# skhu101/SHERF

Hardware: NVIDIA B200
Metric: ray_samples_per_sec (higher is better)
Workload: dtype bf16x3 (bf16 hi/lo split products on tcgen05 kind::f16, 16 significand bits per operand, fp32 accumulate) in every linear layer

## Files before the change

include/sherf_b200.h:

```cpp
#ifndef SHERF_B200_H
#define SHERF_B200_H

#include <stddef.h>
#include <stdint.h>

#ifdef __cplusplus
extern "C" {
#endif

#define SHERF_ABI_VERSION 5
#if defined(__GNUC__)
#define SHERF_API __attribute__((visibility("default")))
#else
#define SHERF_API
#endif
#define SHERF_NUM_JOINTS 24
#define SHERF_NUM_LEVELS 3

enum {
  SHERF_OK = 0,
  SHERF_E_INVALID = -1,
  SHERF_E_SCRATCH = -2,
  SHERF_E_CUDA = -3,
  SHERF_E_UNSUPPORTED = -4
// ... 237 lines not shown
                                            int32_t* bins_out , void* stream);

SHERF_API int sherf_debug_linear(int precision, const float* A, int lda, const float* W, const float* bias, float* Y, int ldy,
                                 int M, int N, int K, int act, void* scratch, size_t scratch_bytes, void* stream);

SHERF_API void sherf_debug_set_trace(long long* device_buf);

SHERF_API const char* sherf_last_error(void);
SHERF_API int sherf_abi_version(void);
SHERF_API int64_t sherf_last_launch_count(void);
SHERF_API int64_t sherf_last_importance_point_count(void);
SHERF_API void sherf_set_profiling(int enabled);
SHERF_API float sherf_last_stage_ms(int stage);
SHERF_API float sherf_last_host_us(int part);
SHERF_API int sherf_nn_list_stats(double* out);

#ifdef __cplusplus
}
#endif
#endif
```

sherf_b200/_lib.py:

```python
from __future__ import annotations

import ctypes as C
import os

from . import build as _build

c_float_p = C.c_void_p
c_int_p = C.c_void_p

MLP_FP32, MLP_TF32, MLP_TF32X3, MLP_BF16X3 = 0, 1, 2, 3
ABI_VERSION = 5


class SherfSmplModel(C.Structure):
    _fields_ = [('v_template', c_float_p), ('shapedirs', c_float_p), ('posedirs', c_float_p), ('j_regressor', c_float_p),
                ('weights', c_float_p), ('parents', C.c_int32 * 24), ('n_verts', C.c_int32)]


class SherfPose(C.Structure):
    _fields_ = [('poses', c_float_p), ('shapes', c_float_p), ('R', c_float_p), ('Th', c_float_p)]


class SherfFrame(C.Structure):
    _fields_ = [('target', SherfPose), ('canonical', SherfPose), ('obs', SherfPose), ('vertices', c_float_p),
# ... 63 lines not shown


class SherfSparseEncoderGrads(C.Structure):
    _fields_ = [('weight', c_float_p * 13), ('bn_weight', c_float_p * 13), ('bn_bias', c_float_p * 13)]


class SherfObservation(C.Structure):
    _fields_ = [('obs', SherfPose), ('canonical', SherfPose), ('obs_vertices', c_float_p), ('t_vertices', c_float_p), ('obs_K', c_float_p),
                ('obs_R', c_float_p), ('obs_T', c_float_p), ('faces', c_int_p), ('last_face', c_int_p), ('n_faces', C.c_int32),
                ('reserved', C.c_int32), ('obs_img', c_float_p), ('img_h', C.c_int32), ('img_w', C.c_int32), ('obs_feat', c_float_p),
                ('feat_ch', C.c_int32), ('feat_h', C.c_int32), ('feat_w', C.c_int32), ('reserved2', C.c_int32), ('proj_w', c_float_p),
                ('proj_b', c_float_p)]


EXPORTS = ['sherf_render_backward_after_forward', 'sherf_sparse_encoder_train_scratch_bytes', 'sherf_sparse_encode_train', 'sherf_sparse_encode_backward', 'sherf_prepare_observation_backward', 'sherf_backward_scratch_bytes', 'sherf_render_backward', 'sherf_smpl_vertices', 'sherf_count_survivors', 'sherf_observation_scratch_bytes', 'sherf_prepare_observation', 'sherf_debug_set_trace', 'sherf_sparse_encoder_scratch_bytes', 'sherf_sparse_encode', 'sherf_generate_rays', 'sherf_debug_sample_importance', 'sherf_debug_linear', 'sherf_scratch_bytes', 'sherf_render_forward', 'sherf_lbs_transforms', 'sherf_depth_range', 'sherf_last_error',
           'sherf_abi_version', 'sherf_last_launch_count', 'sherf_last_importance_point_count', 'sherf_set_profiling', 'sherf_last_stage_ms', 'sherf_last_host_us', 'sherf_nn_list_stats']

_lib = None


def lib_path() -> str:
    return _build.LIB_PATH


def load():
    global _lib
    if _lib is not None:
        return _lib
    path = lib_path()
    if not os.path.exists(path):
        raise RuntimeError(f'{path} not found: build it with `python -m sherf_b200.build` (or __graft_entry__.build()); '
# ... 53 lines not shown
    lib.sherf_observation_scratch_bytes.restype = C.c_size_t
    lib.sherf_observation_scratch_bytes.argtypes = [C.c_int32]
    lib.sherf_prepare_observation.restype = C.c_int
    lib.sherf_prepare_observation.argtypes = [C.POINTER(SherfSmplModel), C.POINTER(SherfObservation), C.c_void_p, C.c_void_p, C.c_void_p,
                                              C.c_void_p, C.POINTER(C.c_int32), C.c_void_p, C.c_void_p, C.c_size_t, C.c_void_p]
    lib.sherf_debug_set_trace.argtypes = [C.c_void_p]
    lib.sherf_last_error.restype = C.c_char_p
    lib.sherf_abi_version.restype = C.c_int
    lib.sherf_last_launch_count.restype = C.c_int64
    lib.sherf_last_importance_point_count.restype = C.c_int64
    lib.sherf_set_profiling.argtypes = [C.c_int]
    lib.sherf_last_stage_ms.restype = C.c_float
    lib.sherf_last_stage_ms.argtypes = [C.c_int]
    lib.sherf_nn_list_stats.restype = C.c_int
    lib.sherf_nn_list_stats.argtypes = [C.POINTER(C.c_double)]
    lib.sherf_last_host_us.restype = C.c_float
    lib.sherf_last_host_us.argtypes = [C.c_int]
    if lib.sherf_abi_version() != ABI_VERSION:
        raise RuntimeError('libsherf_b200.so ABI version mismatch')
    _lib = lib
    return lib


def check(rc: int):
    if rc != 0:
        raise RuntimeError(f'sherf_b200 error {rc}: {load().sherf_last_error().decode()}')
```

sherf_b200/csrc/api.cu:

```cuda
#include "common.cuh"
#include "stages.cuh"
#include <cstdarg>
#include <cstdio>
#include <cstring>
#include <cstdlib>
#include <vector>
#include <chrono>

namespace sherf {

thread_local LaunchCounter g_launches;
thread_local bool g_pack_plan_only = false;
static thread_local char g_err[512] = "";
static thread_local int64_t g_last_launches = 0;
static thread_local int64_t g_last_fine_points = 0;
static thread_local int g_profiling = 0;
static thread_local float g_stage_ms[8] = {0, 0, 0, 0, 0, 0, 0, 0};
static thread_local FrameTables g_last_ft{};
static thread_local float g_host_us[4] = {0, 0, 0, 0};
static inline double now_us() { return std::chrono::duration<double, std::micro>(std::chrono::steady_clock::now().time_since_epoch()).count(); }

void set_error(const char* fmt, ...) {
  va_list ap;
  va_start(ap, fmt);
  vsnprintf(g_err, sizeof(g_err), fmt, ap);
  va_end(ap);
}

constexpr int kMaxCell = 1 << 18;

bool nn_lists_enabled() {
  const char* e = getenv("SHERF_NN_LEGACY");
  return !(e && atoi(e) != 0);
}
int nn_list_cap() {
  const char* e = getenv("SHERF_NN_LIST_CAP");
  const int k = e ? atoi(e) : kNnlCap;
  return k < 1 ? 1 : (k > kNnlCap ? kNnlCap : k);
}
static size_t chunk_cap_limit() {
  static size_t cap = 0;
  if (!cap) {
    const char* e = getenv("SHERF_CHUNK_CAP");
    const long v = e ? atol(e) : 0;
    cap = v >= 128 ? (size_t)(v / 128 * 128) : (size_t)(1 << 19);
  }
  return cap;
}

struct Arena {
  char* base; size_t size; size_t off; bool dry;
  template <typename T> T* take(size_t n) {
    off = (off + 255) & ~(size_t)255;
// ... 7 lines not shown
  FrameTables ft;
  float* planes_cl; float* feat_cl; float* vol_cl[3];
  int* sample_vid; int* ray_count; int* block_sums; int* ray_start; int64_t* total;
  int* point_sample; int* point_vid;
  float* sigma; float* rgb;
  float* fine_depths; int* sample_vid_f; int* ray_count_f; int* ray_start_f; int64_t* total_f; int* point_sample_f; int* point_vid_f;
  float* sigma_f; float* rgb_f;
  float* packed_w;
  float* canon_w;
  unsigned char* fused_blob; float* fused_bias; float* xf_blob; float* ff_blob;
  unsigned char* pp_blob; float* pp_bias; unsigned char* pp_xv;
  unsigned char* xb_blob; unsigned char* fr_blob;
  float* chunk;
  float* gather2;
  float* lbs_joints; float* lbs_pf;
};

static int chunk_cap(int N, int S, int SF) {
  const size_t NS = (size_t)N * (S > SF ? S : SF);
  return (int)((NS < chunk_cap_limit()) ? ((NS + 127) / 128 * 128) : chunk_cap_limit());
}

static size_t carve(Arena& a, const SherfScene& sc, int N, int S, int SF, int V, Layout& L) {
  const size_t NS = (size_t)N * S, NF = (size_t)N * SF;
  FrameTables& ft = L.ft;
  ft.fc = a.take<FrameConst>(1);
  ft.A = a.take<float>(3 * kJoints * 16);
  ft.joints = a.take<float>(3 * kJoints * 3);
  ft.posefeat = a.take<float>(3 * kPoseFeat);
  ft.poff = a.take<float>((size_t)3 * V * 3);
  ft.soff = a.take<float>((size_t)2 * V * 3);
  ft.verts_smpl = a.take<float>((size_t)V * 3);
  ft.T1 = a.take<VertexWarp>(V);
  ft.T3 = a.take<VertexWarp>(V);
  ft.g1_cell_start = a.take<int>(kMaxCell + 1);
  ft.g3_cell_start = a.take<int>(kMaxCell + 1);
  ft.g_cursor = a.take<int>((size_t)2 * kMaxCell);
  ft.g_block_sums = a.take<int>((size_t)2 * (kMaxCell / 1024 + 2));
  ft.g_total = a.take<int64_t>(2);
  ft.g1_verts = a.take<float4>(V);
  ft.g3_verts = a.take<float4>(V);
  ft.g1_occ = a.take<unsigned char>(kMaxCell);
  ft.maxcell = kMaxCell;
  ft.nnl_on = nn_lists_enabled() ? 1 : 0;
  ft.nnl_cap = nn_list_cap();
  ft.nnl_count = a.take<int>(4);
  ft.nnl_cand = a.take<unsigned char>((size_t)kMaxCell * kNnlSub3);
  for (int g = 0; g < 2; ++g) {
    ft.nnl_slot[g] = a.take<int>(kMaxCell);
    ft.nnl_slot_cell[g] = a.take<int>(kNnlSlots);
    ft.nnl_len[g] = a.take<int>((size_t)kNnlSlots * kNnlSub3);
    ft.nnl_ent[g] = a.take<float4>((size_t)kNnlSlots * kNnlSub3 * kNnlCap);
  }
  L.lbs_joints = a.take<float>(kJoints * 3);
  L.lbs_pf = a.take<float>(kPoseFeat);
  L.planes_cl = a.take<float>((size_t)3 * sc.plane_ch * sc.plane_h * sc.plane_w);
  L.feat_cl = a.take<float>((size_t)sc.feat_ch * sc.feat_h * sc.feat_w);
  for (int l = 0; l < 3; ++l)
    L.vol_cl[l] = a.take<float>((size_t)sc.vol_ch[l] * sc.vol_dim[l][0] * sc.vol_dim[l][1] * sc.vol_dim[l][2]);
  L.sample_vid = a.take<int>(NS);
// ... 190 lines not shown
    SHERF_CUDA_OK(cudaMemcpy(len.data(), ft.nnl_len[g], sizeof(int) * (size_t)nsub, cudaMemcpyDeviceToHost));
    double sum = 0.0, mx = 0.0, over = 0.0;
    for (int i = 0; i < nsub; ++i) {
      if (len[i] < 0) over += 1.0;
      else { sum += len[i]; mx = len[i] > mx ? len[i] : mx; }
    }
    out[1 + 4 * g] = nsub;
    out[2 + 4 * g] = nsub > over ? sum / (nsub - over) : 0.0;
    out[3 + 4 * g] = mx;
    out[4 + 4 * g] = nsub ? over / nsub : 0.0;
  }
  out[9] = ft.nnl_cap;
  return SHERF_OK;
}

size_t sherf_scratch_bytes(const SherfScene* scene, int32_t n_rays, int32_t n_samples, int32_t n_importance, int32_t n_verts) {
  if (!scene || n_rays <= 0 || n_samples < 2 || n_importance < 0 || n_verts <= 0) return 0;
  Arena a{nullptr, 0, 0, true};
  Layout L;
  return carve(a, *scene, n_rays, n_samples, n_importance, n_verts, L) + 512;
}

static int validate(const SherfSmplModel* smpl, const SherfFrame* fr, const SherfScene* sc, const SherfWeights* w,
                    const SherfRays* rays, const SherfOptions* opts, const SherfOut* out) {
  if (!smpl || !fr || !sc || !w || !rays || !opts || !out) { set_error("null argument struct"); return SHERF_E_INVALID; }
  if (rays->n_rays <= 0 || rays->n_samples < 2 || rays->n_samples > 256) {
    set_error("n_rays must be > 0 and 2 <= n_samples <= 256 (got %d, %d)", rays->n_rays, rays->n_samples);
    return SHERF_E_INVALID;
  }
  if ((int64_t)rays->n_rays * rays->n_samples >= (1LL << 31)) { set_error("n_rays * n_samples must be < 2^31"); return SHERF_E_INVALID; }
// ... 32 lines not shown

int sherf_render_forward(const SherfSmplModel* smpl, const SherfFrame* frame, const SherfScene* scene,
                         const SherfWeights* weights, const SherfRays* rays, const SherfOptions* opts, const SherfOut* out,
                         const SherfDebug* dbg, void* scratch, size_t scratch_bytes, void* stream, int64_t* n_points_out) {
  g_err[0] = 0;
  const double t_enter = now_us();
  RC(validate(smpl, frame, scene, weights, rays, opts, out));
  const int N = rays->n_rays, S = rays->n_samples, SF = rays->n_importance, V = smpl->n_verts;
  cudaStream_t st = (cudaStream_t)stream;
  Arena a{(char*)scratch, scratch_bytes, 0, false};
  const size_t mis = ((size_t)a.base) & 255;
  if (mis) { a.base += 256 - mis; a.size -= 256 - mis; }
  Layout L;
  const size_t need = carve(a, *scene, N, S, SF, V, L);
  if (!scratch || need > a.size) { set_error("scratch arena too small: need %zu bytes, have %zu", need, scratch_bytes); return SHERF_E_SCRATCH; }
  g_launches.n = 0;
  g_last_fine_points = 0;
  StageTimer tm;
  tm.init(g_profiling != 0, st);
  g_tm = &tm;
  struct Guard {
    cudaStream_t st; bool forked = false, joined = false;
    ~Guard() {
      g_tm = nullptr;
      if (forked && !joined && g_side.s) { cudaEventRecord(g_side.ldone, g_side.s); cudaStreamWaitEvent(st, g_side.ldone, 0); }
    }
  } guard;
  guard.st = st;

  const bool side = !getenv("SHERF_NO_PROLOGUE_OVERLAP") && g_side.ensure() == 0;
// ... 548 lines not shown
```

sherf_b200/csrc/common.cuh:

```cuda
#pragma once
#include <cuda_runtime.h>
#include <stdint.h>
#include <stddef.h>
#include <string.h>
#include "../../include/sherf_b200.h"

namespace sherf {

constexpr int kJoints = 24;
constexpr int kPoseFeat = 207;
constexpr float kPi2 = 1.57079632679489661923f;

struct GridDesc {
  float origin[3];
  float inv_cell;
  float cell;
  int dim[3];
  int ncell;
};

constexpr int kNnlSub = 2;
constexpr int kNnlSub3 = kNnlSub * kNnlSub * kNnlSub;
constexpr int kNnlCap = 64;
constexpr int kNnlSlots = 6144;

struct NnLists {
  const int* slot;
  const int* len;
  const float4* ent;
  const unsigned char* cand;
};

__device__ __forceinline__ bool nnl_cell(const GridDesc& g, float qx, float qy, float qz, int& cell, int& sub) {
  const float tx = (qx - g.origin[0]) * g.inv_cell, ty = (qy - g.origin[1]) * g.inv_cell, tz = (qz - g.origin[2]) * g.inv_cell;
  const int cx = (int)floorf(tx), cy = (int)floorf(ty), cz = (int)floorf(tz);
  if (cx < 0 || cx >= g.dim[0] || cy < 0 || cy >= g.dim[1] || cz < 0 || cz >= g.dim[2]) return false;
  cell = (cz * g.dim[1] + cy) * g.dim[0] + cx;
  const int sx = min((int)((tx - (float)cx) * (float)kNnlSub), kNnlSub - 1);
  const int sy = min((int)((ty - (float)cy) * (float)kNnlSub), kNnlSub - 1);
  const int sz = min((int)((tz - (float)cz) * (float)kNnlSub), kNnlSub - 1);
  sub = (sz * kNnlSub + sy) * kNnlSub + sx;
  return true;
}

__device__ __forceinline__ int nnl_index(const GridDesc& g, const int* __restrict__ slot, float qx, float qy, float qz) {
  int cell, sub;
  if (!nnl_cell(g, qx, qy, qz, cell, sub)) return -1;
  const int sl = slot[cell];
  return sl < 0 ? sl - 1 : sl * kNnlSub3 + sub;
}

struct __align__(16) VertexWarp {
  float Rinv[9];
  float t[3];
  float off0[3];
  float off1[3];
  float off2[3];
  float Af[12];
  float pad[3];
};
static_assert(sizeof(VertexWarp) == 36 * 4, "VertexWarp must be 144 B");

struct FrameConst {
  float R_tgt[9], Th_tgt[3];
// ... 84 lines not shown
  int* g_cursor;
  int* g_block_sums;
  int64_t* g_total;
  float4* g1_verts;
  float4* g3_verts;
  unsigned char* g1_occ;
  int maxcell;
  int nnl_on;
  int nnl_cap;
  int* nnl_slot[2];
  int* nnl_slot_cell[2];
  int* nnl_count;
  int* nnl_len[2];
  float4* nnl_ent[2];
  unsigned char* nnl_cand;
  NnLists lists(int g) const {
    return nnl_on ? NnLists{nnl_slot[g], nnl_len[g], nnl_ent[g], g == 0 ? nnl_cand : nullptr} : NnLists{nullptr, nullptr, nullptr, nullptr};
  }
};
bool nn_lists_enabled();
int nn_list_cap();

int run_prologue_frame(const SherfFrame& frame, const FrameTables& ft, cudaStream_t st);
int run_prologue_cull(const SherfSmplModel& smpl, const SherfFrame& frame, const SherfRays& rays, const SherfOptions& opts,
                      const FrameTables& ft, cudaStream_t st);
int run_prologue_tables(const SherfSmplModel& smpl, const SherfFrame& frame, const FrameTables& ft, cudaStream_t st);
int run_lbs_only(const SherfSmplModel& smpl, const SherfPose& pose, float* A_out, float* joints_tmp, float* pf_tmp, cudaStream_t st);
int run_depth_range(const SherfRays& rays, FrameConst* fc, cudaStream_t st);
int run_exclusive_scan(const int* cnt, int n, int* block_sums, int* start, int64_t* total_dev, cudaStream_t st);

}
```

sherf_b200/csrc/cull.cu:

```cuda
#include "common.cuh"

namespace sherf {

__device__ __forceinline__ void nn_27(const GridDesc& g, const int* __restrict__ cell_start, const float4* __restrict__ gv,
                                      float qx, float qy, float qz, int cx, int cy, int cz, float& best, int& best_id) {
  const int x0 = max(cx - 1, 0), x1 = min(cx + 1, g.dim[0] - 1);
  for (int z = max(cz - 1, 0); z <= min(cz + 1, g.dim[2] - 1); ++z) {
    for (int y = max(cy - 1, 0); y <= min(cy + 1, g.dim[1] - 1); ++y) {
      const int row = (z * g.dim[1] + y) * g.dim[0];
      const int b = cell_start[row + x0], e = cell_start[row + x1 + 1];
      for (int k = b; k < e; ++k) {
        const float4 v = gv[k];
        const float d2 = dist2_xyz(qx, qy, qz, v.x, v.y, v.z);
        const int id = __float_as_int(v.w);
        if (d2 < best || (d2 == best && id < best_id)) { best = d2; best_id = id; }
      }
    }
  }
}

__device__ __forceinline__ void cull_query(const FrameConst& fc, const float* __restrict__ origins, const float* __restrict__ dirs, int n,
                                           float t, float q[3]) {
  float p[3];
  p[0] = __fsub_rn(mul_add_sep(t, dirs[n * 3], origins[n * 3]), fc.Th_tgt[0]);
// ... 84 lines not shown
  __syncthreads();
  const GridDesc& g = fc.g1;
  const int count = *queue_count;
  if (cand_out && blockIdx.x == 0 && threadIdx.x == 0) *cand_out = count;
  for (int j = blockIdx.x * blockDim.x + threadIdx.x; j < count; j += gridDim.x * blockDim.x) {
    const int s = queue[j];
    const int n = s / S, i = s - n * S;
    const float t = depths ? depths[s] : sample_depth(nearv[n], farv[n], i, S);
    float q[3];
    cull_query(fc, origins, dirs, n, t, q);
    float best = 3.0e38f;
    int bid = 0x7fffffff;
    const float qx = q[0], qy = q[1], qz = q[2];
    const int li = nl.slot ? nnl_index(g, nl.slot, qx, qy, qz) : -1;
    const int ln = li >= 0 ? nl.len[li] : -1;
    if (ln >= 0) {
      const float4* e = nl.ent + (size_t)li * kNnlCap;
      for (int k = 0; k < ln; ++k) {
        const float4 v = e[k];
        const float d2 = dist2_xyz(qx, qy, qz, v.x, v.y, v.z);
        const int id = __float_as_int(v.w);
        if (d2 < best || (d2 == best && id < bid)) { best = d2; bid = id; }
      }
    } else {
      const int cx = grid_coord(q[0], g.origin[0], g.inv_cell, g.dim[0]);
      const int cy = grid_coord(q[1], g.origin[1], g.inv_cell, g.dim[1]);
      const int cz = grid_coord(q[2], g.origin[2], g.inv_cell, g.dim[2]);
      nn_27(g, cell_start, gv, qx, qy, qz, cx, cy, cz, best, bid);
    }
    const int vid = best < thr ? bid : -1;
// ... 107 lines not shown
```

sherf_b200/csrc/front_fused.cu:

```cuda
#include "common.cuh"
#include "stages.cuh"
#include "umma.cuh"
#include <cuda_bf16.h>
#include <cstdlib>

namespace sherf {

namespace fr {
constexpr uint32_t kLboA = 2080;
constexpr uint32_t kChunkHalf = 4 * kLboA;
constexpr uint32_t kChunk = 2 * kChunkHalf;
constexpr int kSlots = 3;
constexpr uint32_t kLboF = 2048;
constexpr uint32_t kF3d = kSlots * kChunk;
constexpr uint32_t kWr = kF3d + 12 * kLboF;
constexpr uint32_t kWrBlock = 4096;
constexpr uint32_t kWp = kWr + 3 * kWrBlock;
constexpr uint32_t kWpStage = 12288;
constexpr uint32_t kSmemBytes = kWp + 2 * kWpStage;
constexpr uint32_t kD1 = 0, kD2 = 96, kF3dLo = 192;
constexpr int kThreads = 512;
}

struct FrontArgs {
// ... 184 lines not shown
        const int k3 = l4 < 3 ? l4 : 0;
        const float ck = k3 == 0 ? cn[0] : (k3 == 1 ? cn[1] : cn[2]);
        const float gnv = ((ck - fc.spb_min[k3]) / 0.005f) / fc.out_sh[2 - k3] * 2.f - 1.f;
        const float cnv = 2.f * (ck - fc.twb_min[k3]) / (fc.twb_max[k3] - fc.twb_min[k3]) - 1.f;
        if (l4 < 3) { s_pt[gi][l4] = gnv; s_pt[gi][3 + l4] = cnv; }
        pu = u; pv = v;
      }
      if (act) {
        if (l4 < 3) {
          P.geo[(size_t)lp * 8 + l4] = l4 == 0 ? cn[0] : (l4 == 1 ? cn[1] : cn[2]);
          P.geo[(size_t)lp * 8 + 3 + l4] = l4 == 0 ? cdir[0] : (l4 == 1 ? cdir[1] : cdir[2]);
        } else {
          P.geo[(size_t)lp * 8 + 6] = 0.f;
          P.geo[(size_t)lp * 8 + 7] = 0.f;
        }
        if (DBG && l4 == 0 && gp < P.dbg_max) {
          if (P.dbg_vid3) P.dbg_vid3[gp] = vid3;
          if (P.dbg_can) { P.dbg_can[gp * 3] = cn[0]; P.dbg_can[gp * 3 + 1] = cn[1]; P.dbg_can[gp * 3 + 2] = cn[2]; }
          if (P.dbg_cdir) { P.dbg_cdir[gp * 3] = cdir[0]; P.dbg_cdir[gp * 3 + 1] = cdir[1]; P.dbg_cdir[gp * 3 + 2] = cdir[2]; }
          if (P.dbg_uv) { P.dbg_uv[gp * 2] = u; P.dbg_uv[gp * 2 + 1] = v; }
        }
      }
    }
    __syncwarp();

    int offT[2] = {-1, -1}, offI = -1;
    float wT[2] = {0.f, 0.f}, wI = 0.f;
    const float* pt = s_pt[gi];
#pragma unroll 1
    for (int c = 0; c < 12; ++c) {
// ... 248 lines not shown
  if (G.np <= 0) return SHERF_OK;
  if (!G.t_vertices) { set_error("internal: the front kernel needs the seeded canonical-vertex search"); return SHERF_E_INVALID; }
  FrontArgs a;
  a.G = G; a.wblob = blob; a.bp = w.proj_b; a.br = w.reproj_b; a.tok = tok;
  { const char* e = getenv("SHERF_FRONT_KNOCK"); a.knock = e ? atoi(e) : 0; }
  static bool attr_done = false;
  static int num_sms = 148;
  if (!attr_done) {
    SHERF_CUDA_OK(cudaFuncSetAttribute(k_front_fused<false>, cudaFuncAttributeMaxDynamicSharedMemorySize, (int)fr::kSmemBytes));
    SHERF_CUDA_OK(cudaFuncSetAttribute(k_front_fused<true>, cudaFuncAttributeMaxDynamicSharedMemorySize, (int)fr::kSmemBytes));
    int dev = 0;
    SHERF_CUDA_OK(cudaGetDevice(&dev));
    SHERF_CUDA_OK(cudaDeviceGetAttribute(&num_sms, cudaDevAttrMultiProcessorCount, dev));
    attr_done = true;
  }
  const bool dbg = G.dbg_feat || G.dbg_vid3 || G.dbg_can || G.dbg_cdir || G.dbg_uv;
  const int ntiles = (G.np + 127) / 128;
  const int grid = ntiles < 2 * num_sms ? ntiles : 2 * num_sms;
  if (dbg) k_front_fused<true><<<grid, fr::kThreads, fr::kSmemBytes, st>>>(a);
  else k_front_fused<false><<<grid, fr::kThreads, fr::kSmemBytes, st>>>(a);
  SHERF_LAUNCH_CHECK();
  return SHERF_OK;
}

}
```

sherf_b200/csrc/gather.cu:

```cuda
#include "common.cuh"
#include "stages.cuh"
#include <cstdlib>

namespace sherf {

struct ClJobs { const float* in[8]; float* out[8]; int C[8]; long long M[8]; int blk0[9]; int vec[8]; int n; };

__global__ void __launch_bounds__(256) k_to_channels_last(const ClJobs J) {
  __shared__ float tile[32][129];
  int j = 0;
  while (j + 1 < J.n && (int)blockIdx.x >= J.blk0[j + 1]) ++j;
  const float* __restrict__ in = J.in[j];
  float* __restrict__ out = J.out[j];
  const int C = J.C[j];
  const int64_t M = J.M[j];
  const int cblocks = (C + 31) / 32;
  const int lb = (int)blockIdx.x - J.blk0[j];
  const int64_t m0 = (int64_t)(lb / cblocks) * 128;
  const int c0 = (lb % cblocks) * 32;
  const int tid = threadIdx.x;
  if (J.vec[j]) {
#pragma unroll
    for (int k = 0; k < 4; ++k) {
      const int idx = tid + 256 * k, r = idx >> 5, q = idx & 31;
// ... 584 lines not shown
              const float4 val = off[tp] >= 0 ? __ldg(reinterpret_cast<const float4*>(vol + off[tp] + 32 * gsel)) : make_float4(0.f, 0.f, 0.f, 0.f);
              acc.x += val.x * w[tp]; acc.y += val.y * w[tp]; acc.z += val.z * w[tp]; acc.w += val.w * w[tp];
            }
            if (active) *reinterpret_cast<float4*>(f3 + coff + 32 * gsel + c4) = acc;
            if (DBG && dbgf && active) *reinterpret_cast<float4*>(dbgf + 192 + coff + 32 * gsel + c4) = acc;
          }
        }
        coff += 32 * (l + 1);
      }
    }
    if (active && !BWD) {
      float gval = 0.f;
      if (l8 == 0) gval = can[0]; else if (l8 == 1) gval = can[1]; else if (l8 == 2) gval = can[2];
      else if (l8 == 3) gval = cdir[0]; else if (l8 == 4) gval = cdir[1]; else if (l8 == 5) gval = cdir[2];
      P.geo[(size_t)lp * 8 + l8] = gval;
      if (DBG && l8 == 0 && gp < P.dbg_max) {
        if (P.dbg_vid3) P.dbg_vid3[gp] = vid3;
        if (P.dbg_can) { P.dbg_can[gp * 3] = can[0]; P.dbg_can[gp * 3 + 1] = can[1]; P.dbg_can[gp * 3 + 2] = can[2]; }
        if (P.dbg_cdir) { P.dbg_cdir[gp * 3] = cdir[0]; P.dbg_cdir[gp * 3 + 1] = cdir[1]; P.dbg_cdir[gp * 3 + 2] = cdir[2]; }
        if (P.dbg_uv) { P.dbg_uv[gp * 2] = u; P.dbg_uv[gp * 2 + 1] = v; }
      }
    }
  }
}


int run_point_gather(const GatherParams& P, cudaStream_t st) {
  if (P.np <= 0) return SHERF_OK;
  const bool dbg = P.dbg_feat || P.dbg_vid3 || P.dbg_can || P.dbg_cdir || P.dbg_uv;
  if (getenv("SHERF_GATHER_V1")) {
    const int blocks = min(ceil_div(P.np, 8), 148 * 16);
    k_point_gather<<<blocks, 256, 0, st>>>(P);
  } else {
    const int blocks = min(ceil_div(P.np, 32), 148 * 8);
    if (dbg) k_point_gather4<true, false><<<blocks, 256, 0, st>>>(P);
    else k_point_gather4<false, false><<<blocks, 256, 0, st>>>(P);
  }
  SHERF_LAUNCH_CHECK();
  return SHERF_OK;
}

int run_point_scatter(const GatherParams& P, cudaStream_t st) {
  if (P.np <= 0) return SHERF_OK;
  const int blocks = min(ceil_div(P.np, 32), 148 * 8);
// ... 7 lines not shown
```

sherf_b200/csrc/prologue.cu:

```cuda
#include "common.cuh"
#include <limits.h>

namespace sherf {

__global__ void k_joints(const float* __restrict__ vt, const float* __restrict__ sd, const float* __restrict__ jr,
                         const float* __restrict__ b0, const float* __restrict__ b1, const float* __restrict__ b2,
                         int V, float* __restrict__ joints) {
  const int j = blockIdx.x, s = blockIdx.y;
  const float* beta = s == 0 ? b0 : (s == 1 ? b1 : b2);
  float b[10];
#pragma unroll
  for (int k = 0; k < 10; ++k) b[k] = beta[k];
  float acc[3] = {0.f, 0.f, 0.f};
  for (int v = threadIdx.x; v < V; v += blockDim.x) {
    float w = jr[(size_t)j * V + v];
    if (w != 0.f) {
#pragma unroll
      for (int c = 0; c < 3; ++c) {
        const float* row = sd + ((size_t)v * 3 + c) * 10;
        float off = 0.f;
#pragma unroll
        for (int k = 0; k < 10; ++k) off += row[k] * b[k];
        acc[c] += w * (vt[v * 3 + c] + off);
      }
// ... 324 lines not shown
    const unsigned act = __activemask(), m = __ballot_sync(act, any);
    const int lane = threadIdx.x & 31, leader = __ffs(act) - 1;
    int base = 0;
    if (lane == leader && m) base = atomicAdd(nslots, __popc(m));
    base = __shfl_sync(act, base, leader);
    int s = -1;
    if (any) {
      s = base + __popc(m & ((1u << lane) - 1u));
      if (s < kNnlSlots) slot_cell[s] = c;
      else s = -2;
    }
    slot[c] = s;
  }
}

__global__ void __launch_bounds__(256) k_nnl_build(const FrameConst* __restrict__ fc, int g, const int* __restrict__ start,
                                                   const float4* __restrict__ gv, const int* __restrict__ slot_cell,
                                                   const int* __restrict__ nslots, int cap, float cut, int* __restrict__ len,
                                                   float4* __restrict__ ent, unsigned char* __restrict__ cand) {
  static_assert(kNnlSub == 2, "one bit per axis selects the sub-cell");
  const GridDesc sg = g == 0 ? fc->g1 : fc->g3;
  const int lane = threadIdx.x & 31;
  const int ns = min(*nslots, kNnlSlots);
  const float f = sg.cell * 0.5f, eps = 1.0e-4f * sg.cell;
  for (int sl = (blockIdx.x * blockDim.x + threadIdx.x) >> 5; sl < ns; sl += (gridDim.x * blockDim.x) >> 5) {
    const int c = slot_cell[sl];
    const int cx = c % sg.dim[0], t = c / sg.dim[0], cy = t % sg.dim[1], cz = t / sg.dim[1];
    const int cc[3] = {cx, cy, cz};
    float lo[3][2], hi[3][2], ctr[3][2];
#pragma unroll
    for (int k = 0; k < 3; ++k)
#pragma unroll
      for (int h = 0; h < 2; ++h) {
        lo[k][h] = sg.origin[k] + (float)cc[k] * sg.cell + (float)h * f - eps;
        hi[k][h] = lo[k][h] + f + 2.f * eps;
        ctr[k][h] = 0.5f * (lo[k][h] + hi[k][h]);
      }
    float dc[8];
#pragma unroll
    for (int i = 0; i < 8; ++i) dc[i] = 3.0e38f;
    for (int zz = max(cz - 1, 0); zz <= min(cz + 1, sg.dim[2] - 1); ++zz)
      for (int yy = max(cy - 1, 0); yy <= min(cy + 1, sg.dim[1] - 1); ++yy) {
        const int row = (zz * sg.dim[1] + yy) * sg.dim[0];
        const int b = start[row + max(cx - 1, 0)], e = start[row + min(cx + 1, sg.dim[0] - 1) + 1];
        for (int k = b + lane; k < e; k += 32) {
          const float4 v = gv[k];
          float d[3][2];
#pragma unroll
          for (int h = 0; h < 2; ++h) {
            d[0][h] = (v.x - ctr[0][h]) * (v.x - ctr[0][h]);
            d[1][h] = (v.y - ctr[1][h]) * (v.y - ctr[1][h]);
            d[2][h] = (v.z - ctr[2][h]) * (v.z - ctr[2][h]);
          }
#pragma unroll
          for (int i = 0; i < 8; ++i) dc[i] = fminf(dc[i], d[0][i & 1] + d[1][(i >> 1) & 1] + d[2][i >> 2]);
        }
      }
    float lim2[8];
    int rmax = 0, rbits = 0;
#pragma unroll
    for (int i = 0; i < 8; ++i) {
      float x = dc[i];
      for (int o = 16; o > 0; o >>= 1) x = fminf(x, __shfl_xor_sync(0xffffffffu, x, o));
      float lim = (sqrtf(x) + 1.7320508f * (0.5f * f + eps)) * 1.0001f + eps;
      if (cut > 0.f) lim = fminf(lim, cut);
      const int r = lim < 0.999f * sg.cell ? 1 : (lim < 1.999f * sg.cell ? 2 : 0);
      rmax = max(rmax, r);
      rbits |= r > 0 ? 1 << i : 0;
      lim2[i] = r > 0 ? lim * lim : -1.f;
    }
    int n[8];
#pragma unroll
    for (int i = 0; i < 8; ++i) n[i] = 0;
    float4* out = ent + (size_t)sl * kNnlSub3 * kNnlCap;
    for (int zz = max(cz - rmax, 0); zz <= min(cz + rmax, sg.dim[2] - 1); ++zz)
      for (int yy = max(cy - rmax, 0); yy <= min(cy + rmax, sg.dim[1] - 1); ++yy) {
        const int row = (zz * sg.dim[1] + yy) * sg.dim[0];
        const int b = start[row + max(cx - rmax, 0)], e = start[row + min(cx + rmax, sg.dim[0] - 1) + 1];
        for (int k0 = b; k0 < e; k0 += 32) {
          const int k = k0 + lane;
          const float4 v = k < e ? gv[k] : make_float4(3.0e38f, 3.0e38f, 3.0e38f, 0.f);
          float o[3][2];
#pragma unroll
          for (int h = 0; h < 2; ++h) {
            const float ox = fmaxf(fmaxf(lo[0][h] - v.x, v.x - hi[0][h]), 0.f);
            const float oy = fmaxf(fmaxf(lo[1][h] - v.y, v.y - hi[1][h]), 0.f);
            const float oz = fmaxf(fmaxf(lo[2][h] - v.z, v.z - hi[2][h]), 0.f);
            o[0][h] = ox * ox; o[1][h] = oy * oy; o[2][h] = oz * oz;
          }
#pragma unroll
          for (int i = 0; i < 8; ++i) {
            const bool take = k < e && o[0][i & 1] + o[1][(i >> 1) & 1] + o[2][i >> 2] <= lim2[i];
            const unsigned m = __ballot_sync(0xffffffffu, take);
            const int pos = n[i] + __popc(m & ((1u << lane) - 1u));
            if (take && pos < cap) out[i * kNnlCap + pos] = v;
            n[i] += __popc(m);
          }
        }
      }
#pragma unroll
    for (int i = 0; i < 8; ++i) {
      if (lane == i) {
        const int l = ((rbits >> i) & 1) && n[i] <= cap ? n[i] : -1;
        len[sl * kNnlSub3 + i] = l;
        if (cand) cand[(size_t)c * kNnlSub3 + i] = l != 0;
      }
    }
  }
}

__global__ void k_depth_range(const float* __restrict__ nearv, const float* __restrict__ farv, int N, int S, FrameConst* fc) {
  int lo = INT_MAX, hi = INT_MIN;
  for (int n = blockIdx.x * blockDim.x + threadIdx.x; n < N; n += gridDim.x * blockDim.x) {
    float a = sample_depth(nearv[n], farv[n], 0, S), b = sample_depth(nearv[n], farv[n], S - 1, S);
    int ia = float_to_ordered(a), ib = float_to_ordered(b);
    lo = min(lo, min(ia, ib));
    hi = max(hi, max(ia, ib));
  }
  for (int o = 16; o > 0; o >>= 1) {
    lo = min(lo, __shfl_xor_sync(0xffffffffu, lo, o));
    hi = max(hi, __shfl_xor_sync(0xffffffffu, hi, o));
// ... 38 lines not shown
  SHERF_LAUNCH_CHECK();
  int rc = run_exclusive_scan(counts, ft.maxcell, bsums, g == 0 ? ft.g1_cell_start : ft.g3_cell_start, ft.g_total + g, st);
  if (rc) return rc;
  k_grid_scatter<<<dim3(ceil_div(V, 256), 1), 256, 0, st>>>(ft.verts_smpl, fr.t_vertices, V, ft.fc, ft.g_cursor, ft.maxcell, ft.g1_cell_start,
                                                           ft.g3_cell_start, ft.g1_verts, ft.g3_verts, g);
  SHERF_LAUNCH_CHECK();
  if (g == 0 || lists) {
    k_grid_occupancy<<<ceil_div(ft.maxcell, 256), 256, 0, st>>>(ft.fc, g, g == 0 ? ft.g1_cell_start : ft.g3_cell_start, g == 0 ? ft.g1_occ : nullptr,
                                                                lists ? ft.nnl_slot[g] : nullptr, ft.nnl_slot_cell[g], ft.nnl_count + g,
                                                                lists && g == 0 ? ft.nnl_cand : nullptr);
    SHERF_LAUNCH_CHECK();
  }
  if (lists) {
    const float cut = g == 0 ? 0.05f * 1.0001f + 1.0e-5f : 0.f;
    k_nnl_build<<<148 * 8, 256, 0, st>>>(ft.fc, g, g == 0 ? ft.g1_cell_start : ft.g3_cell_start, g == 0 ? ft.g1_verts : ft.g3_verts,
                                         ft.nnl_slot_cell[g], ft.nnl_count + g, ft.nnl_cap, cut, ft.nnl_len[g], ft.nnl_ent[g],
                                         g == 0 ? ft.nnl_cand : nullptr);
    SHERF_LAUNCH_CHECK();
  }
  return SHERF_OK;
}

int run_prologue_frame(const SherfFrame& fr, const FrameTables& ft, cudaStream_t st) {
  SHERF_CUDA_OK(cudaMemsetAsync(ft.fc, 0, sizeof(FrameConst), st));
  k_frame_const<<<1, 32, 0, st>>>(fr, make_float3((float)fr.out_sh[0], (float)fr.out_sh[1], (float)fr.out_sh[2]), ft.fc);
  SHERF_LAUNCH_CHECK();
  return SHERF_OK;
}

int run_prologue_cull(const SherfSmplModel& smpl, const SherfFrame& fr, const SherfRays& rays, const SherfOptions& opts,
                      const FrameTables& ft, cudaStream_t st) {
  const int V = smpl.n_verts;
// ... 31 lines not shown
```

Before: 5.847 billion.

## Prune dominated vertices from nearest-vertex candidate lists, one warp per sub-cell

Rebuilds the per-sub-cell nearest-vertex candidate lists so that each warp handles one sub-cell instead of all eight. The warp tracks the nearest vertex to each of the sub-cell's eight corners and its centre, then drops any candidate that one of those nine witnesses dominates everywhere in the box. Shorter lists mean fewer distance checks per query in the gather and front stages, at the cost of a heavier build kernel. The change also adds debug query counters and a list-dump API, which only run when debug taps are on.

```diff
diff --git a/include/sherf_b200.h b/include/sherf_b200.h
--- a/include/sherf_b200.h
+++ b/include/sherf_b200.h
@@ -275,6 +275,9 @@
 SHERF_API float sherf_last_stage_ms(int stage);
 SHERF_API float sherf_last_host_us(int part);
 SHERF_API int sherf_nn_list_stats(double* out);
+SHERF_API int sherf_nn_query_stats(double* out);
+SHERF_API int sherf_nn_list_dump(int32_t grid, const int32_t* index, int32_t n, int32_t* cell_out, int32_t* len_out, float* ent_out,
+                                 float* grid_out);
 
 #ifdef __cplusplus
 }
diff --git a/sherf_b200/_lib.py b/sherf_b200/_lib.py
--- a/sherf_b200/_lib.py
+++ b/sherf_b200/_lib.py
@@ -101,7 +101,8 @@
 
 
 EXPORTS = ['sherf_render_backward_after_forward', 'sherf_sparse_encoder_train_scratch_bytes', 'sherf_sparse_encode_train', 'sherf_sparse_encode_backward', 'sherf_prepare_observation_backward', 'sherf_backward_scratch_bytes', 'sherf_render_backward', 'sherf_smpl_vertices', 'sherf_count_survivors', 'sherf_observation_scratch_bytes', 'sherf_prepare_observation', 'sherf_debug_set_trace', 'sherf_sparse_encoder_scratch_bytes', 'sherf_sparse_encode', 'sherf_generate_rays', 'sherf_debug_sample_importance', 'sherf_debug_linear', 'sherf_scratch_bytes', 'sherf_render_forward', 'sherf_lbs_transforms', 'sherf_depth_range', 'sherf_last_error',
-           'sherf_abi_version', 'sherf_last_launch_count', 'sherf_last_importance_point_count', 'sherf_set_profiling', 'sherf_last_stage_ms', 'sherf_last_host_us', 'sherf_nn_list_stats']
+           'sherf_abi_version', 'sherf_last_launch_count', 'sherf_last_importance_point_count', 'sherf_set_profiling', 'sherf_last_stage_ms', 'sherf_last_host_us', 'sherf_nn_list_stats',
+           'sherf_nn_query_stats', 'sherf_nn_list_dump']
 
 _lib = None
 
@@ -185,6 +186,10 @@
     lib.sherf_last_stage_ms.argtypes = [C.c_int]
     lib.sherf_nn_list_stats.restype = C.c_int
     lib.sherf_nn_list_stats.argtypes = [C.POINTER(C.c_double)]
+    lib.sherf_nn_query_stats.restype = C.c_int
+    lib.sherf_nn_query_stats.argtypes = [C.POINTER(C.c_double)]
+    lib.sherf_nn_list_dump.restype = C.c_int
+    lib.sherf_nn_list_dump.argtypes = [C.c_int32, C.c_void_p, C.c_int32, C.c_void_p, C.c_void_p, C.c_void_p, C.c_void_p]
     lib.sherf_last_host_us.restype = C.c_float
     lib.sherf_last_host_us.argtypes = [C.c_int]
     if lib.sherf_abi_version() != ABI_VERSION:
diff --git a/sherf_b200/csrc/api.cu b/sherf_b200/csrc/api.cu
--- a/sherf_b200/csrc/api.cu
+++ b/sherf_b200/csrc/api.cu
@@ -37,6 +37,10 @@
   const char* e = getenv("SHERF_NN_LIST_CAP");
   const int k = e ? atoi(e) : kNnlCap;
   return k < 1 ? 1 : (k > kNnlCap ? kNnlCap : k);
+}
+bool nn_list_prune() {
+  const char* e = getenv("SHERF_NN_PRUNE");
+  return !(e && atoi(e) == 0);
 }
 static size_t chunk_cap_limit() {
   static size_t cap = 0;
@@ -74,6 +78,7 @@
   float* chunk;
   float* gather2;
   float* lbs_joints; float* lbs_pf;
+  unsigned long long* nn_qstat;
 };
 
 static int chunk_cap(int N, int S, int SF) {
@@ -104,6 +109,9 @@
   ft.maxcell = kMaxCell;
   ft.nnl_on = nn_lists_enabled() ? 1 : 0;
   ft.nnl_cap = nn_list_cap();
+  ft.nnl_prune = nn_list_prune() ? 1 : 0;
+  ft.nnl_qstat = nullptr;
+  L.nn_qstat = a.take<unsigned long long>(6);
   ft.nnl_count = a.take<int>(4);
   ft.nnl_cand = a.take<unsigned char>((size_t)kMaxCell * kNnlSub3);
   for (int g = 0; g < 2; ++g) {
@@ -324,6 +332,43 @@
   return SHERF_OK;
 }
 
+int sherf_nn_query_stats(double* out) {
+  if (!out || !g_last_ft.nnl_qstat) { set_error("the last forward on this thread counted no nearest-vertex queries (lists and debug taps needed)"); return SHERF_E_INVALID; }
+  SHERF_CUDA_OK(cudaDeviceSynchronize());
+  unsigned long long q[6];
+  SHERF_CUDA_OK(cudaMemcpy(q, g_last_ft.nnl_qstat, sizeof(q), cudaMemcpyDeviceToHost));
+  for (int i = 0; i < 6; ++i) out[i] = (double)q[i];
+  return SHERF_OK;
+}
+
+int sherf_nn_list_dump(int32_t grid, const int32_t* index, int32_t n, int32_t* cell_out, int32_t* len_out, float* ent_out, float* grid_out) {
+  if (!g_last_ft.nnl_on) { set_error("the last forward on this thread built no candidate lists"); return SHERF_E_INVALID; }
+  if ((grid != 0 && grid != 1) || n < 0 || (n > 0 && (!index || !cell_out || !len_out || !ent_out)) || !grid_out) {
+    set_error("sherf_nn_list_dump: bad arguments");
+    return SHERF_E_INVALID;
+  }
+  const FrameTables& ft = g_last_ft;
+  SHERF_CUDA_OK(cudaDeviceSynchronize());
+  int cnt[4];
+  SHERF_CUDA_OK(cudaMemcpy(cnt, ft.nnl_count, sizeof(cnt), cudaMemcpyDeviceToHost));
+  const int nsub = (cnt[grid] < kNnlSlots ? cnt[grid] : kNnlSlots) * kNnlSub3;
+  FrameConst fc;
+  SHERF_CUDA_OK(cudaMemcpy(&fc, ft.fc, sizeof(fc), cudaMemcpyDeviceToHost));
+  const GridDesc& g = grid == 0 ? fc.g1 : fc.g3;
+  for (int k = 0; k < 3; ++k) { grid_out[k] = g.origin[k]; grid_out[5 + k] = (float)g.dim[k]; }
+  grid_out[3] = g.cell; grid_out[4] = g.inv_cell;
+  for (int i = 0; i < n; ++i) {
+    if (index[i] < 0 || index[i] >= nsub) { set_error("sherf_nn_list_dump: list index %d outside [0, %d)", index[i], nsub); return SHERF_E_INVALID; }
+    int sc = 0;
+    SHERF_CUDA_OK(cudaMemcpy(&sc, ft.nnl_slot_cell[grid] + index[i] / kNnlSub3, sizeof(int), cudaMemcpyDeviceToHost));
+    cell_out[i] = sc;
+    SHERF_CUDA_OK(cudaMemcpy(len_out + i, ft.nnl_len[grid] + index[i], sizeof(int), cudaMemcpyDeviceToHost));
+    SHERF_CUDA_OK(cudaMemcpy(ent_out + (size_t)i * kNnlCap * 4, ft.nnl_ent[grid] + (size_t)index[i] * kNnlCap, sizeof(float4) * kNnlCap,
+                             cudaMemcpyDeviceToHost));
+  }
+  return SHERF_OK;
+}
+
 size_t sherf_scratch_bytes(const SherfScene* scene, int32_t n_rays, int32_t n_samples, int32_t n_importance, int32_t n_verts) {
   if (!scene || n_rays <= 0 || n_samples < 2 || n_importance < 0 || n_verts <= 0) return 0;
   Arena a{nullptr, 0, 0, true};
@@ -386,6 +431,10 @@
   Layout L;
   const size_t need = carve(a, *scene, N, S, SF, V, L);
   if (!scratch || need > a.size) { set_error("scratch arena too small: need %zu bytes, have %zu", need, scratch_bytes); return SHERF_E_SCRATCH; }
+  if (dbg && L.ft.nnl_on) {
+    L.ft.nnl_qstat = L.nn_qstat;
+    SHERF_CUDA_OK(cudaMemsetAsync(L.nn_qstat, 0, sizeof(unsigned long long) * 6, st));
+  }
   g_launches.n = 0;
   g_last_fine_points = 0;
   StageTimer tm;
diff --git a/sherf_b200/csrc/common.cuh b/sherf_b200/csrc/common.cuh
--- a/sherf_b200/csrc/common.cuh
+++ b/sherf_b200/csrc/common.cuh
@@ -29,6 +29,7 @@
   const int* len;
   const float4* ent;
   const unsigned char* cand;
+  unsigned long long* qstat;
 };
 
 __device__ __forceinline__ bool nnl_cell(const GridDesc& g, float qx, float qy, float qz, int& cell, int& sub) {
@@ -48,6 +49,13 @@
   if (!nnl_cell(g, qx, qy, qz, cell, sub)) return -1;
   const int sl = slot[cell];
   return sl < 0 ? sl - 1 : sl * kNnlSub3 + sub;
+}
+
+__device__ __forceinline__ void nn_count_query(const GridDesc& g, const NnLists& nl, float qx, float qy, float qz) {
+  const int li = nl.slot ? nnl_index(g, nl.slot, qx, qy, qz) : -1;
+  const int ln = li >= 0 ? nl.len[li] : -1;
+  atomicAdd(&nl.qstat[ln > 0 ? 0 : 1], 1ull);
+  if (ln > 0) atomicAdd(&nl.qstat[2], (unsigned long long)ln);
 }
 
 struct __align__(16) VertexWarp {
@@ -162,12 +170,16 @@
   int* nnl_len[2];
   float4* nnl_ent[2];
   unsigned char* nnl_cand;
+  int nnl_prune;
+  unsigned long long* nnl_qstat;
   NnLists lists(int g) const {
-    return nnl_on ? NnLists{nnl_slot[g], nnl_len[g], nnl_ent[g], g == 0 ? nnl_cand : nullptr} : NnLists{nullptr, nullptr, nullptr, nullptr};
+    return nnl_on ? NnLists{nnl_slot[g], nnl_len[g], nnl_ent[g], g == 0 ? nnl_cand : nullptr, nnl_qstat ? nnl_qstat + 3 * g : nullptr}
+                  : NnLists{nullptr, nullptr, nullptr, nullptr, nullptr};
   }
 };
 bool nn_lists_enabled();
 int nn_list_cap();
+bool nn_list_prune();
 
 int run_prologue_frame(const SherfFrame& frame, const FrameTables& ft, cudaStream_t st);
 int run_prologue_cull(const SherfSmplModel& smpl, const SherfFrame& frame, const SherfRays& rays, const SherfOptions& opts,
diff --git a/sherf_b200/csrc/cull.cu b/sherf_b200/csrc/cull.cu
--- a/sherf_b200/csrc/cull.cu
+++ b/sherf_b200/csrc/cull.cu
@@ -122,6 +122,10 @@
     const float qx = q[0], qy = q[1], qz = q[2];
     const int li = nl.slot ? nnl_index(g, nl.slot, qx, qy, qz) : -1;
     const int ln = li >= 0 ? nl.len[li] : -1;
+    if (nl.qstat) {
+      atomicAdd(&nl.qstat[ln >= 0 ? 0 : 1], 1ull);
+      if (ln > 0) atomicAdd(&nl.qstat[2], (unsigned long long)ln);
+    }
     if (ln >= 0) {
       const float4* e = nl.ent + (size_t)li * kNnlCap;
       for (int k = 0; k < ln; ++k) {
diff --git a/sherf_b200/csrc/front_fused.cu b/sherf_b200/csrc/front_fused.cu
--- a/sherf_b200/csrc/front_fused.cu
+++ b/sherf_b200/csrc/front_fused.cu
@@ -222,6 +222,7 @@
           P.geo[(size_t)lp * 8 + 6] = 0.f;
           P.geo[(size_t)lp * 8 + 7] = 0.f;
         }
+        if (DBG && l4 == 0 && P.nl3.qstat) nn_count_query(fc.g3, P.nl3, cn[0], cn[1], cn[2]);
         if (DBG && l4 == 0 && gp < P.dbg_max) {
           if (P.dbg_vid3) P.dbg_vid3[gp] = vid3;
           if (P.dbg_can) { P.dbg_can[gp * 3] = cn[0]; P.dbg_can[gp * 3 + 1] = cn[1]; P.dbg_can[gp * 3 + 2] = cn[2]; }
@@ -500,7 +501,7 @@
     SHERF_CUDA_OK(cudaDeviceGetAttribute(&num_sms, cudaDevAttrMultiProcessorCount, dev));
     attr_done = true;
   }
-  const bool dbg = G.dbg_feat || G.dbg_vid3 || G.dbg_can || G.dbg_cdir || G.dbg_uv;
+  const bool dbg = G.dbg_feat || G.dbg_vid3 || G.dbg_can || G.dbg_cdir || G.dbg_uv || G.nl3.qstat;
   const int ntiles = (G.np + 127) / 128;
   const int grid = ntiles < 2 * num_sms ? ntiles : 2 * num_sms;
   if (dbg) k_front_fused<true><<<grid, fr::kThreads, fr::kSmemBytes, st>>>(a);
diff --git a/sherf_b200/csrc/gather.cu b/sherf_b200/csrc/gather.cu
--- a/sherf_b200/csrc/gather.cu
+++ b/sherf_b200/csrc/gather.cu
@@ -622,6 +622,7 @@
       if (l8 == 0) gval = can[0]; else if (l8 == 1) gval = can[1]; else if (l8 == 2) gval = can[2];
       else if (l8 == 3) gval = cdir[0]; else if (l8 == 4) gval = cdir[1]; else if (l8 == 5) gval = cdir[2];
       P.geo[(size_t)lp * 8 + l8] = gval;
+      if (DBG && l8 == 0 && P.nl3.qstat) nn_count_query(fc.g3, P.nl3, can[0], can[1], can[2]);
       if (DBG && l8 == 0 && gp < P.dbg_max) {
         if (P.dbg_vid3) P.dbg_vid3[gp] = vid3;
         if (P.dbg_can) { P.dbg_can[gp * 3] = can[0]; P.dbg_can[gp * 3 + 1] = can[1]; P.dbg_can[gp * 3 + 2] = can[2]; }
@@ -635,7 +636,7 @@
 
 int run_point_gather(const GatherParams& P, cudaStream_t st) {
   if (P.np <= 0) return SHERF_OK;
-  const bool dbg = P.dbg_feat || P.dbg_vid3 || P.dbg_can || P.dbg_cdir || P.dbg_uv;
+  const bool dbg = P.dbg_feat || P.dbg_vid3 || P.dbg_can || P.dbg_cdir || P.dbg_uv || P.nl3.qstat;
   if (getenv("SHERF_GATHER_V1")) {
     const int blocks = min(ceil_div(P.np, 8), 148 * 16);
     k_point_gather<<<blocks, 256, 0, st>>>(P);
diff --git a/sherf_b200/csrc/prologue.cu b/sherf_b200/csrc/prologue.cu
--- a/sherf_b200/csrc/prologue.cu
+++ b/sherf_b200/csrc/prologue.cu
@@ -362,97 +362,134 @@
   }
 }
 
-__global__ void __launch_bounds__(256) k_nnl_build(const FrameConst* __restrict__ fc, int g, const int* __restrict__ start,
-                                                   const float4* __restrict__ gv, const int* __restrict__ slot_cell,
-                                                   const int* __restrict__ nslots, int cap, float cut, int* __restrict__ len,
+__device__ __forceinline__ bool nnl_dominated(const float4* __restrict__ dom, const float L[3], const float H[3], float4 v) {
+  const float x[3] = {v.x, v.y, v.z};
+  float dv = 0.f;
+#pragma unroll
+  for (int k = 0; k < 3; ++k) dv += fmaxf(__fmul_rn(L[k] - x[k], L[k] - x[k]), __fmul_rn(H[k] - x[k], H[k] - x[k]));
+  for (int j = 0; j < 9; ++j) {
+    const float4 w = dom[j];
+    const float wk[3] = {w.x, w.y, w.z};
+    float sa = 0.f, sb = 0.f;
+#pragma unroll
+    for (int k = 0; k < 3; ++k) {
+      const float q = x[k] > wk[k] ? H[k] : L[k];
+      const float a = __fsub_rn(q, wk[k]), b = __fsub_rn(q, x[k]);
+      sa = __fadd_rn(sa, __fmul_rn(a, a));
+      sb = __fadd_rn(sb, __fmul_rn(b, b));
+    }
+    if (__fsub_rn(sa, sb) < -1.0e-5f * (w.w + dv)) return true;
+  }
+  return false;
+}
+
+__global__ void __launch_bounds__(256, 4) k_nnl_build(const FrameConst* __restrict__ fc, int g, const int* __restrict__ start,
+                                                   const float4* __restrict__ gv, const float* __restrict__ pv, const int* __restrict__ slot_cell,
+                                                   const int* __restrict__ nslots, int cap, float cut, int prune, int* __restrict__ len,
                                                    float4* __restrict__ ent, unsigned char* __restrict__ cand) {
   static_assert(kNnlSub == 2, "one bit per axis selects the sub-cell");
+  __shared__ float4 sdom[8][9];
   const GridDesc sg = g == 0 ? fc->g1 : fc->g3;
   const int lane = threadIdx.x & 31;
-  const int ns = min(*nslots, kNnlSlots);
+  float4* dom = sdom[threadIdx.x >> 5];
+  const int nl = min(*nslots, kNnlSlots) * kNnlSub3;
   const float f = sg.cell * 0.5f, eps = 1.0e-4f * sg.cell;
-  for (int sl = (blockIdx.x * blockDim.x + threadIdx.x) >> 5; sl < ns; sl += (gridDim.x * blockDim.x) >> 5) {
+  for (int li = (blockIdx.x * blockDim.x + threadIdx.x) >> 5; li < nl; li += (gridDim.x * blockDim.x) >> 5) {
+    const int sl = li / kNnlSub3, i = li % kNnlSub3;
     const int c = slot_cell[sl];
     const int cx = c % sg.dim[0], t = c / sg.dim[0], cy = t % sg.dim[1], cz = t / sg.dim[1];
-    const int cc[3] = {cx, cy, cz};
-    float lo[3][2], hi[3][2], ctr[3][2];
-#pragma unroll
-    for (int k = 0; k < 3; ++k)
-#pragma unroll
-      for (int h = 0; h < 2; ++h) {
-        lo[k][h] = sg.origin[k] + (float)cc[k] * sg.cell + (float)h * f - eps;
-        hi[k][h] = lo[k][h] + f + 2.f * eps;
-        ctr[k][h] = 0.5f * (lo[k][h] + hi[k][h]);
-      }
-    float dc[8];
-#pragma unroll
-    for (int i = 0; i < 8; ++i) dc[i] = 3.0e38f;
+    const int cc[3] = {cx, cy, cz}, sb[3] = {i & 1, (i >> 1) & 1, i >> 2};
+    float lo[3], hi[3], ctr[3], lat[3][2];
+#pragma unroll
+    for (int k = 0; k < 3; ++k) {
+      lo[k] = sg.origin[k] + (float)cc[k] * sg.cell + (float)sb[k] * f - eps;
+      hi[k] = lo[k] + f + 2.f * eps;
+      ctr[k] = 0.5f * (lo[k] + hi[k]);
+#pragma unroll
+      for (int h = 0; h < 2; ++h) lat[k][h] = sg.origin[k] + (float)cc[k] * sg.cell + (float)(sb[k] + h) * f;
+    }
+    float dl[9];
+    int il[9];
+#pragma unroll
+    for (int j = 0; j < 9; ++j) { dl[j] = 3.0e38f; il[j] = 0x7fffffff; }
     for (int zz = max(cz - 1, 0); zz <= min(cz + 1, sg.dim[2] - 1); ++zz)
       for (int yy = max(cy - 1, 0); yy <= min(cy + 1, sg.dim[1] - 1); ++yy) {
         const int row = (zz * sg.dim[1] + yy) * sg.dim[0];
         const int b = start[row + max(cx - 1, 0)], e = start[row + min(cx + 1, sg.dim[0] - 1) + 1];
         for (int k = b + lane; k < e; k += 32) {
           const float4 v = gv[k];
-          float d[3][2];
-#pragma unroll
-          for (int h = 0; h < 2; ++h) {
-            d[0][h] = (v.x - ctr[0][h]) * (v.x - ctr[0][h]);
-            d[1][h] = (v.y - ctr[1][h]) * (v.y - ctr[1][h]);
-            d[2][h] = (v.z - ctr[2][h]) * (v.z - ctr[2][h]);
+          const int id = __float_as_int(v.w);
+          const float p[3] = {v.x, v.y, v.z};
+          float d[3], a[3][2];
+#pragma unroll
+          for (int q = 0; q < 3; ++q) {
+            d[q] = (p[q] - ctr[q]) * (p[q] - ctr[q]);
+#pragma unroll
+            for (int h = 0; h < 2; ++h) a[q][h] = (p[q] - lat[q][h]) * (p[q] - lat[q][h]);
           }
 #pragma unroll
-          for (int i = 0; i < 8; ++i) dc[i] = fminf(dc[i], d[0][i & 1] + d[1][(i >> 1) & 1] + d[2][i >> 2]);
-        }
-      }
-    float lim2[8];
-    int rmax = 0, rbits = 0;
-#pragma unroll
-    for (int i = 0; i < 8; ++i) {
-      float x = dc[i];
-      for (int o = 16; o > 0; o >>= 1) x = fminf(x, __shfl_xor_sync(0xffffffffu, x, o));
-      float lim = (sqrtf(x) + 1.7320508f * (0.5f * f + eps)) * 1.0001f + eps;
-      if (cut > 0.f) lim = fminf(lim, cut);
-      const int r = lim < 0.999f * sg.cell ? 1 : (lim < 1.999f * sg.cell ? 2 : 0);
-      rmax = max(rmax, r);
-      rbits |= r > 0 ? 1 << i : 0;
-      lim2[i] = r > 0 ? lim * lim : -1.f;
-    }
-    int n[8];
-#pragma unroll
-    for (int i = 0; i < 8; ++i) n[i] = 0;
-    float4* out = ent + (size_t)sl * kNnlSub3 * kNnlCap;
-    for (int zz = max(cz - rmax, 0); zz <= min(cz + rmax, sg.dim[2] - 1); ++zz)
-      for (int yy = max(cy - rmax, 0); yy <= min(cy + rmax, sg.dim[1] - 1); ++yy) {
-        const int row = (zz * sg.dim[1] + yy) * sg.dim[0];
-        const int b = start[row + max(cx - rmax, 0)], e = start[row + min(cx + rmax, sg.dim[0] - 1) + 1];
-        for (int k0 = b; k0 < e; k0 += 32) {
-          const int k = k0 + lane;
-          const float4 v = k < e ? gv[k] : make_float4(3.0e38f, 3.0e38f, 3.0e38f, 0.f);
-          float o[3][2];
-#pragma unroll
-          for (int h = 0; h < 2; ++h) {
-            const float ox = fmaxf(fmaxf(lo[0][h] - v.x, v.x - hi[0][h]), 0.f);
-            const float oy = fmaxf(fmaxf(lo[1][h] - v.y, v.y - hi[1][h]), 0.f);
-            const float oz = fmaxf(fmaxf(lo[2][h] - v.z, v.z - hi[2][h]), 0.f);
-            o[0][h] = ox * ox; o[1][h] = oy * oy; o[2][h] = oz * oz;
-          }
-#pragma unroll
-          for (int i = 0; i < 8; ++i) {
-            const bool take = k < e && o[0][i & 1] + o[1][(i >> 1) & 1] + o[2][i >> 2] <= lim2[i];
-            const unsigned m = __ballot_sync(0xffffffffu, take);
-            const int pos = n[i] + __popc(m & ((1u << lane) - 1u));
-            if (take && pos < cap) out[i * kNnlCap + pos] = v;
-            n[i] += __popc(m);
+          for (int j = 0; j < 9; ++j) {
+            const float x = j < 8 ? a[0][j & 1] + a[1][(j >> 1) & 1] + a[2][j >> 2] : d[0] + d[1] + d[2];
+            if (x < dl[j] || (x == dl[j] && id < il[j])) { dl[j] = x; il[j] = id; }
           }
         }
       }
 #pragma unroll
-    for (int i = 0; i < 8; ++i) {
-      if (lane == i) {
-        const int l = ((rbits >> i) & 1) && n[i] <= cap ? n[i] : -1;
-        len[sl * kNnlSub3 + i] = l;
-        if (cand) cand[(size_t)c * kNnlSub3 + i] = l != 0;
+    for (int j = 0; j < 9; ++j)
+      for (int o = 16; o > 0; o >>= 1) {
+        const float od = __shfl_xor_sync(0xffffffffu, dl[j], o);
+        const int oi = __shfl_xor_sync(0xffffffffu, il[j], o);
+        if (od < dl[j] || (od == dl[j] && oi < il[j])) { dl[j] = od; il[j] = oi; }
       }
+    float lim = (sqrtf(dl[8]) + 1.7320508f * (0.5f * f + eps)) * 1.0001f + eps;
+    if (cut > 0.f) lim = fminf(lim, cut);
+    const int r = lim < 0.999f * sg.cell ? 1 : (lim < 1.999f * sg.cell ? 2 : 0);
+    const float lim2 = lim * lim;
+    int n = 0;
+    if (r > 0) {
+      if (prune) {
+        int id = il[8];
+#pragma unroll
+        for (int j = 0; j < 8; ++j)
+          if (lane == j) id = il[j];
+        __syncwarp();
+        if (lane < 9) {
+          const float w[3] = {pv[(size_t)id * 3], pv[(size_t)id * 3 + 1], pv[(size_t)id * 3 + 2]};
+          float dw = 0.f;
+#pragma unroll
+          for (int k = 0; k < 3; ++k) dw += fmaxf(__fmul_rn(lo[k] - w[k], lo[k] - w[k]), __fmul_rn(hi[k] - w[k], hi[k] - w[k]));
+          dom[lane] = make_float4(w[0], w[1], w[2], dw);
+        }
+        __syncwarp();
+      }
+      float4* out = ent + (size_t)li * kNnlCap;
+      for (int zz = max(cz - r, 0); zz <= min(cz + r, sg.dim[2] - 1); ++zz)
+        for (int yy = max(cy - r, 0); yy <= min(cy + r, sg.dim[1] - 1); ++yy) {
+          const int row = (zz * sg.dim[1] + yy) * sg.dim[0];
+          const int b = start[row + max(cx - r, 0)], e = start[row + min(cx + r, sg.dim[0] - 1) + 1];
+          for (int k0 = b; k0 < e; k0 += 32) {
+            const int k = k0 + lane;
+            bool take = false;
+            float4 v;
+            if (k < e) {
+              v = gv[k];
+              const float ox = fmaxf(fmaxf(lo[0] - v.x, v.x - hi[0]), 0.f);
+              const float oy = fmaxf(fmaxf(lo[1] - v.y, v.y - hi[1]), 0.f);
+              const float oz = fmaxf(fmaxf(lo[2] - v.z, v.z - hi[2]), 0.f);
+              take = ox * ox + oy * oy + oz * oz <= lim2;
+              if (take && prune) take = !nnl_dominated(dom, lo, hi, v);
+            }
+            const unsigned m = __ballot_sync(0xffffffffu, take);
+            const int pos = n + __popc(m & ((1u << lane) - 1u));
+            if (take && pos < cap) out[pos] = v;
+            n += __popc(m);
+          }
+        }
+    }
+    if (lane == 0) {
+      const int l = r > 0 && n <= cap ? n : -1;
+      len[li] = l;
+      if (cand) cand[(size_t)c * kNnlSub3 + i] = l != 0;
     }
   }
 }
@@ -521,8 +558,8 @@
   if (lists) {
     const float cut = g == 0 ? 0.05f * 1.0001f + 1.0e-5f : 0.f;
     k_nnl_build<<<148 * 8, 256, 0, st>>>(ft.fc, g, g == 0 ? ft.g1_cell_start : ft.g3_cell_start, g == 0 ? ft.g1_verts : ft.g3_verts,
-                                         ft.nnl_slot_cell[g], ft.nnl_count + g, ft.nnl_cap, cut, ft.nnl_len[g], ft.nnl_ent[g],
-                                         g == 0 ? ft.nnl_cand : nullptr);
+                                         g == 0 ? ft.verts_smpl : fr.t_vertices, ft.nnl_slot_cell[g], ft.nnl_count + g, ft.nnl_cap, cut,
+                                         ft.nnl_prune, ft.nnl_len[g], ft.nnl_ent[g], g == 0 ? ft.nnl_cand : nullptr);
     SHERF_LAUNCH_CHECK();
   }
   return SHERF_OK;
```

Result: faster. 5.955 billion (median of 6 runs) (+1.8%).
